# hbdat/cvpr22_cross_modal_pseudo_labeling

Measured on AMD Instinct MI355X. Metric: images/sec student-teacher train step (COCO 800x1333), higher is better.
Workload: dtype f32 (bf16x3 split MFMA, fp32 accum); 1 GPU; student_teacher_mask_rcnn_uncertainty.yaml R-50-C4, 2 img/GPU 3x800x1333, fwd+bwd+allreduce+SGD; global_batch=2, parallelism=dp1, losses_finite=True, pipelined=True

## Files before the change

### cvpr22_cross_modal_pseudo_labeling_amd/_C.py

```python
import contextlib
import functools
import ctypes
import threading

import torch

from . import _cpu, _lib

_L = _lib.load()


def _stream():
    return torch._C._cuda_getCurrentRawStream(torch.cuda.current_device())


class _Same:

    def __enter__(self):
        return None

    def __exit__(self, *exc):
        return False


# ... 737 lines not shown
        raise RuntimeError("im2col_nchw_pair: contiguous [N,C,H,W] float32 HIP tensor expected")
    n, c, h, w = x.shape
    ho, wo = (h + 2 * pad - kh) // stride + 1, (w + 2 * pad - kw) // stride + 1
    kp = -(-(kh * kw * c) // 32) * 32
    out = torch.empty((n * ho * wo, 2 * kp), dtype=torch.bfloat16, device=x.device)
    if out.numel():
        with _on(x.device):
            rc = _L.ovis_im2col_nchw_pair_f32(x.data_ptr(), out.data_ptr(), n, c, h, w, kh, kw, stride, pad, kp, _stream())
        _lib.check(rc, "im2col_nchw_pair")
    return out, (ho, wo)


_GEMM_TLS = threading.local()


@contextlib.contextmanager
def co_scheduled(on=True):
    prev = getattr(_GEMM_TLS, "co", False)
    _GEMM_TLS.co = bool(on)
    try:
        yield
    finally:
        _GEMM_TLS.co = prev


@functools.lru_cache(maxsize=None)
def _gemm_ws_bytes(m, n, ch, ch2, kh, kw, w, config):
    return int(_L.ovis_split_gemm_pair_workspace_bytes_ex(m, n, ch, ch2, kh, kw, w, config))


@functools.lru_cache(maxsize=None)
def _tn_slices(m, n, ch, taps):
    return int(_L.ovis_split_gemm_tn_slices(m, n, ch, taps))


@functools.lru_cache(maxsize=None)
def _gemm_f32_ws_bytes(m, n, k):
    return int(_L.ovis_gemm_f32_workspace_bytes(m, n, k))


@functools.lru_cache(maxsize=None)
def _nms_presorted_ws_bytes(n, k):
    return int(_L.ovis_nms_presorted_workspace_bytes(n, k))


@functools.lru_cache(maxsize=None)
def _topk_ws_bytes(n, a):
    return int(_L.ovis_topk_sorted_workspace_bytes(n, a))


def _gemm_cfg(config):
    return config | (0x10000 if getattr(_GEMM_TLS, "co", False) else 0)


def split_gemm_pair(a_pair, b_pair, bias=None, residual=None, relu=False, out_f32=True, out_pair=False, conv=None,
                    config=0, a2_pair=None, residual_pair=None):
    for t, name in ((a_pair, "a_pair"), (b_pair, "b_pair")) + (((a2_pair, "a2_pair"),) if a2_pair is not None else ()):
        if not (t.is_cuda and t.dtype == torch.bfloat16 and t.dim() == 2 and t.stride(1) == 1):
            raise RuntimeError(f"split_gemm_pair: {name} must be a 2-D bfloat16 HIP tensor in pair layout")
    m, ch = a_pair.shape[0], a_pair.shape[1] // 2
    n, k = b_pair.shape[0], b_pair.shape[1] // 2
    ch2 = 0
    if a2_pair is not None:
        if conv is not None or a2_pair.shape[0] != m:
            raise RuntimeError("split_gemm_pair: a2_pair needs a plain product and as many rows as a_pair")
        ch2 = a2_pair.shape[1] // 2
# ... 148 lines not shown
                                              0 if cp is None else cp.data_ptr(), 4 * n, residual_pair.data_ptr(),
                                              2 * residual_pair.stride(0), gate_pair.data_ptr(), 2 * gate_pair.stride(0), m, n,
                                              ch, config, _stream())
    _lib.check(rc, "split_gemm_pair_rp_gated")
    return c, cp


def split_gemm_pair_tn_supported(n, ch, conv=None):
    if n % 128 or ch % 128:
        return False
    if conv is not None:
        h, w, kh, kw = conv
        return kh % 2 == 1 and kw % 2 == 1
    return True


def split_gemm_pair_tn(g_pair, x_pair, conv=None, scale=None, weight_shape=None):
    for t, name in ((g_pair, "g_pair"), (x_pair, "x_pair")):
        if not (t.is_cuda and t.dtype == torch.bfloat16 and t.dim() == 2 and t.stride(1) == 1):
            raise RuntimeError(f"split_gemm_pair_tn: {name} must be a 2-D bfloat16 HIP tensor in pair layout")
    m, n, ch = g_pair.shape[0], g_pair.shape[1] // 2, x_pair.shape[1] // 2
    if x_pair.shape[0] != m:
        raise RuntimeError("split_gemm_pair_tn: row counts differ")
    h = w = 0
    kh = kw = 1
    if conv is not None:
        h, w, kh, kw = conv
        if m % (h * w):
            raise RuntimeError("split_gemm_pair_tn: rows must be a multiple of h*w")
    dev = g_pair.device
    if m == 0:
        z = torch.zeros((n, kh * kw * ch), dtype=torch.float32, device=dev)
        return z if weight_shape is None else z.new_zeros(weight_shape)
    slices = _tn_slices(m, n, ch, kh * kw)
    slabs = torch.empty((slices, n, kh * kw * ch), dtype=torch.float32, device=dev)
    with _on(dev):
        rc = _L.ovis_split_gemm_pair_tn(g_pair.data_ptr(), 2 * g_pair.stride(0), x_pair.data_ptr(), 2 * x_pair.stride(0),
                                        slabs.data_ptr(), slices, m, n, ch, kh, kw, h, w, _stream())
        _lib.check(rc, "split_gemm_pair_tn")
        if weight_shape is None:
            return slabs[0] if slices == 1 else slabs.sum(0)
        if tuple(weight_shape) != (n, ch, kh, kw):
            raise RuntimeError("split_gemm_pair_tn: weight_shape must be (N, ch, kh, kw)")
        dw = torch.empty(weight_shape, dtype=torch.float32, device=dev)
        if scale is not None:
            scale = _dev(scale.detach(), "scale")
        rc = _L.ovis_slab_reduce_f32(slabs.data_ptr(), 0 if scale is None else scale.data_ptr(), dw.data_ptr(), slices, n,
                                     ch, kh * kw, _stream())
    _lib.check(rc, "slab_reduce")
    return dw


def bias_act_(y, bias=None, residual=None, relu=True):
    if not (y.is_cuda and y.dtype == torch.float32 and y.dim() == 2 and y.is_contiguous()):
        raise RuntimeError("bias_act_: contiguous 2-D float32 HIP tensor expected")
    if residual is not None and not (residual.is_contiguous() and residual.shape == y.shape):
        raise RuntimeError("bias_act_: residual must be contiguous with y's shape")
    if y.numel() == 0:
        return y
    with _on(y.device):
        rc = _L.ovis_bias_act_f32(y.data_ptr(), 0 if bias is None else bias.data_ptr(),
                                  0 if residual is None else residual.data_ptr(), y.shape[0], y.shape[1],
                                  int(bool(relu)), _stream())
    _lib.check(rc, "bias_act")
    return y


# ... 552 lines not shown
```

### cvpr22_cross_modal_pseudo_labeling_amd/_lib.py

```python
import ctypes
import os

_HERE = os.path.dirname(os.path.abspath(__file__))
LIB_PATH = os.path.join(_HERE, "libovis_hip.so")

OVIS_OK = 0
_ERRORS = {-1: "OVIS_EINVAL (bad size or null pointer)",
           -2: "OVIS_ENOSPC (workspace too small)",
           -3: "OVIS_ERANGE (problem size not supported by the kernel)"}

_vp, _i, _f, _sz, _l = ctypes.c_void_p, ctypes.c_int, ctypes.c_float, ctypes.c_size_t, ctypes.c_long

SIGNATURES = {
    "ovis_version": (ctypes.c_char_p, []),
    "ovis_roi_align_forward_f32": (_i, [_vp, _vp, _vp, _i, _i, _i, _i, _i, _i, _i, _f, _i, _vp]),
    "ovis_roi_align_forward_workspace_bytes": (_sz, [_i, _i, _i]),
    "ovis_roi_align_forward_mfma_supported": (_i, [_i, _i, _i, _i]),
    "ovis_roi_align_forward_ws_f32": (_i, [_vp, _vp, _vp, _i, _i, _i, _i, _i, _i, _i, _f, _i, _vp, _sz, _vp]),
    "ovis_roi_align_forward_strided_from_nhwc_f32": (_i, [_vp, _vp, _vp, _i, _i, _i, _i, _i, _i, _i, _i, _f, _i, _i, _vp]),
    "ovis_roi_align_backward_f32": (_i, [_vp, _vp, _vp, _i, _i, _i, _i, _i, _i, _i, _f, _i, _vp]),
    "ovis_roi_align_backward_workspace_bytes": (_sz, [_i, _i, _i, _i]),
    "ovis_roi_align_backward_plane_supported": (_i, [_i, _i, _i, _i]),
    "ovis_roi_align_backward_ws_f32": (_i, [_vp, _vp, _vp, _i, _i, _i, _i, _i, _i, _i, _f, _i, _vp, _sz, _vp]),
    "ovis_roi_align_backward_strided_ws_f32": (_i, [_vp, _vp, _vp, _i, _i, _i, _i, _i, _i, _i, _i, _f, _i, _vp, _sz, _vp]),
# ... 3 lines not shown
    "ovis_roi_pool_backward_f32": (_i, [_vp, _vp, _vp, _vp, _i, _i, _i, _i, _i, _i, _i, _vp]),
    "ovis_deform_psroi_pool_forward_f32": (_i, [_vp] * 5 + [_i] * 7 + [_f] + [_i] * 5 + [_f, _vp]),
    "ovis_deform_psroi_pool_backward_f32": (_i, [_vp] * 7 + [_i] * 7 + [_f] + [_i] * 5 + [_f, _vp]),
    "ovis_nms_workspace_bytes": (_sz, [_i]),
    "ovis_nms_f32": (_i, [_vp, _vp, _i, _f, _i, _vp, _sz, _vp, _vp, _vp]),
    "ovis_nms_grouped_f32": (_i, [_vp, _vp, _vp, _i, _f, _i, _vp, _sz, _vp, _vp, _vp]),
    "ovis_sample_fg_bg": (_i, [_vp, _i, _i, _i, ctypes.c_uint64, _vp, _vp, _vp, _vp]),
    "ovis_project_pasted_masks_f32": (_i, [_vp, _vp, _vp, _vp, _i, _i, _i, _i, _i, _f, _vp, _vp]),
    "ovis_paste_masks_u8": (_i, [_vp, _vp, _i, _i, _i, _i, _f, _vp, _vp]),
    "ovis_render_instances_u8": (_i, [_vp, _i, _i, _vp, _vp, _i, _i, _vp, _vp, _vp, _f, _vp, _i, _vp, _vp]),
    "ovis_nms_presorted_workspace_bytes": (_sz, [_i, _i]),
    "ovis_nms_presorted_batched_f32": (_i, [_vp, _vp, _i, _i, _f, _i, _i, _vp, _sz, _vp, _vp, _vp]),
    "ovis_box_decode_f32": (_i, [_vp, _l, _vp, _l, _l, _i, _f, _f, _f, _f, _f, _i, _vp, _vp, _vp, _vp]),
    "ovis_smooth_l1_picked_fwd_bwd_f32": (_i, [_vp, _l, _i, _i, _vp, _l, _vp, _vp, _i, _i, _f, _f, _vp, _vp, _vp]),
    "ovis_gather_rows": (_i, [_vp, _i, _vp, _vp, _vp, _vp, _vp, _vp, _vp, _vp, _vp]),
    "ovis_rois_from_boxes_f32": (_i, [_vp, _vp, _vp, _i, _vp, _vp]),
    "ovis_deform_conv_implicit_f32": (_i, [_vp, _vp, _vp, _vp, _l, _vp, _vp, _l] + [_i] * 16 + [_vp]),
    "ovis_topk_sorted_workspace_bytes": (_sz, [_i, _i]),
    "ovis_topk_sorted_f32": (_i, [_vp, _l, _i, _i, _i, _vp, _vp, _vp, _sz, _vp]),
    "ovis_rpn_decode_f32": (_i, [_vp, _l, _l, _l, _vp, _vp, _vp, _i, _i, _i, _i, _f, _f, _f, _f, _f, _f, _f, _vp, _vp, _vp]),
    "ovis_sigmoid_focal_loss_forward_f32": (_i, [_vp, _vp, _vp, _i, _i, _f, _f, _vp]),
    "ovis_sigmoid_focal_loss_backward_f32": (_i, [_vp, _vp, _vp, _vp, _i, _i, _f, _f, _vp]),
    "ovis_split_bf16x3_f32": (_i, [_vp, _l, _vp, _l, _i, _i, _vp]),
    "ovis_im2col_split_bf16x3_f32": (_i, [_vp, _vp, _l, _i, _i, _i, _i, _i, _i, _vp]),
    "ovis_bias_act_f32": (_i, [_vp, _vp, _vp, _l, _i, _i, _vp]),
    "ovis_split_pair_f32": (_i, [_vp, _l, _vp, _l, _i, _vp]),
    "ovis_gate_split_pair_rows_f32": (_i, [_vp, _l, _vp, _i, _vp, _vp, _l, _i, _vp, _i, _vp, _vp, _vp]),
    "ovis_gate_split_pair_f32": (_i, [_vp, _l, _vp, _i, _vp, _vp, _l, _i, _vp, _i, _vp]),
    "ovis_im2col_nchw_pair_f32": (_i, [_vp, _vp] + [_i] * 9 + [_vp]),
    "ovis_weight_prep_pair_f32": (_i, [_vp, _vp, _vp, _vp, _i, _i, _i, _vp]),
    "ovis_slab_reduce_f32": (_i, [_vp, _vp, _vp, _i, _i, _i, _i, _vp]),
    "ovis_im2col_pair": (_i, [_vp, _vp, _l, _i, _i, _i, _i, _i, _vp]),
    "ovis_split_gemm_tn_slices": (_i, [_l, _i, _i, _i]),
    "ovis_split_gemm_pair_tn": (_i, [_vp, _l, _vp, _l, _vp, _i, _l, _i, _i, _i, _i, _i, _i, _vp]),
    "ovis_split_gemm_pair_gated": (_i, [_vp, _l, _vp, _l, _vp, _l, _vp, _l, _vp, _l, _l] + [_i] * 8 + [_vp]),
    "ovis_split_gemm_pair_gated_ws": (_i, [_vp, _l, _vp, _l, _vp, _l, _vp, _l, _vp, _l, _l] + [_i] * 7 + [_vp, _sz, _i, _vp]),
    "ovis_split_gemm_pair_workspace_bytes": (_sz, [_l, _i, _i, _i, _i, _i, _i]),
    "ovis_split_gemm_pair_workspace_bytes_ex": (_sz, [_l, _i, _i, _i, _i, _i, _i, _i]),
    "ovis_split_gemm_pair_rp_gated": (_i, [_vp, _l, _vp, _l, _vp, _l, _vp, _l, _vp, _l, _vp, _l, _l, _i, _i, _i, _vp]),
    "ovis_split_gemm_pair_pool_supported": (_i, [_l, _i, _i, _i]),
    "ovis_split_gemm_pair_rp_pool": (_i, [_vp, _l, _vp, _l, _vp, _l, _vp, _l, _vp, _vp, _l, _l, _i, _i, _i, _vp, _i, _f, _vp]),
    "ovis_split_gemm_pair_rp": (_i, [_vp, _l, _vp, _l, _vp, _l, _vp, _l, _vp, _vp, _l, _l, _i, _i, _i, _vp, _sz, _i, _vp]),
    "ovis_split_gemm_pair": (_i, [_vp, _l, _vp, _l, _vp, _l, _vp, _l, _vp, _l, _vp, _vp, _l, _l] + [_i] * 9
                             + [_vp, _sz, _i, _vp]),
    "ovis_match_encode_f32": (_i, [_vp, _vp, _vp, _i, _i, _f, _f, _i, _f, _f, _f, _f, _vp, _vp, _vp, _vp]),
    "ovis_rpn_match_encode_f32": (_i, [_vp, _vp, _vp, _i, _i, _f, _f, _i, _f, _f, _f, _f, _vp, _vp, _vp, _vp]),
    "ovis_project_masks_f32": (_i, [_vp, _vp, _vp, _i, _i, _i, _i, _i, _vp, _vp]),
    "ovis_gemm_f32": (_i, [_vp, _l, _l, _vp, _l, _l, _vp, _vp, _l, _i, _i, _i, _vp]),
    "ovis_gemm_ex_f32": (_i, [_vp, _l, _l, _vp, _l, _l, _vp, _i, _f, _i, _vp, _l, _i, _i, _i, _vp]),
    "ovis_gemm_f32_workspace_bytes": (_sz, [_i, _i, _i]),
    "ovis_gemm_ex_ws_f32": (_i, [_vp, _l, _l, _vp, _l, _l, _vp, _i, _f, _i, _vp, _l, _i, _i, _i, _vp, _sz, _vp]),
    "ovis_deform_im2col_f32": (_i, [_vp, _vp, _vp, _vp] + [_i] * 13 + [_vp]),
    "ovis_deform_col2im_f32": (_i, [_vp, _vp, _vp, _vp] + [_i] * 13 + [_vp]),
    "ovis_deform_col2im_coord_f32": (_i, [_vp, _vp, _vp, _vp, _vp, _vp] + [_i] * 13 + [_vp]),
    "ovis_deform_im2col_pair_rows_f32": (_i, [_vp, _vp, _vp, _vp, _l] + [_i] * 15 + [_vp]),
    "ovis_deform_col2im_rows_f32": (_i, [_vp, _l, _vp, _vp, _vp, _vp, _vp, _vp] + [_i] * 15 + [_vp]),
    "ovis_region_noun_align_f32": (_i, [_vp, _vp, _vp, _vp, _vp, _i, _i, _i, _vp]),
    "ovis_text_embed_f32": (_i, [_vp, _l, _i, _vp, _vp, _i, _i, _vp, _vp]),
    "ovis_project_polygon_masks_f32": (_i, [_vp, _vp, _vp, _vp, _vp, _i, _i, _i, _i, _vp, _vp]),
    "ovis_polygons_to_masks_workspace_bytes": (_sz, [_i, _i, _i]),
    "ovis_polygons_to_masks_u8": (_i, [_vp, _vp, _vp, _i, _i, _i, _i, _vp, _sz, _vp, _vp]),
    "ovis_transform_images_workspace_bytes": (_sz, [_i, _i, _i]),
    "ovis_transform_images_u8": (_i, [_vp, _l, _vp, _i, _i, _i, _vp, _vp, _i, _i, _i, _vp, _sz, _vp, _vp]),
    "ovis_sgd_momentum_multi_f32": (_i, [_vp, _vp, _i, _f, _f, _f, _i, _vp]),
    "ovis_bottleneck_identity_backward_workspace_bytes": (_sz, [_l, _i, _i, _i, _i, _i, _i]),
    "ovis_bottleneck_identity_backward": (_i, [_vp, _l] * 7 + [_vp] * 3 + [_l, _i, _i, _i, _i, _i, _i] + [_vp] * 7 + [_sz, _i, _vp, _vp]),
# ... 38 lines not shown
```

### cvpr22_cross_modal_pseudo_labeling_amd/csrc/bottleneck_backward.hip

```cpp
#include "ovis_common.h"

namespace {

inline size_t bb_align(size_t v) { return (v + 255) & ~(size_t)255; }

struct BbPlan {
  size_t chain_bytes;
  size_t slab_bytes;
  int s1, s2, s3;
};

BbPlan bb_plan(long m, int cin, int mid, int kh, int kw, int width, int config) {
  BbPlan p;
  const size_t a = ovis_split_gemm_pair_workspace_bytes_ex(m, mid, cin, 0, 1, 1, 0, config);
  const size_t b = ovis_split_gemm_pair_workspace_bytes_ex(m, mid, mid, 0, kh, kw, width, config);
  p.chain_bytes = bb_align(a > b ? a : b);
  p.s3 = ovis_split_gemm_tn_slices(m, cin, mid, 1);
  p.s2 = ovis_split_gemm_tn_slices(m, mid, mid, kh * kw);
  p.s1 = ovis_split_gemm_tn_slices(m, mid, cin, 1);
  const size_t w3 = (size_t)p.s3 * cin * mid * 4, w2 = (size_t)p.s2 * mid * mid * kh * kw * 4, w1 = (size_t)p.s1 * mid * cin * 4;
  size_t mx = w3 > w2 ? w3 : w2;
  if (w1 > mx) mx = w1;
  p.slab_bytes = bb_align(mx);
  return p;
}

hipEvent_t* bb_events() {
  static hipEvent_t ev[4];
  static bool made = false;
  if (!made) {
    for (int i = 0; i < 4; ++i)
      if (hipEventCreateWithFlags(&ev[i], hipEventDisableTiming) != hipSuccess) return nullptr;
    made = true;
  }
  return ev;
}

}

extern "C" size_t ovis_bottleneck_identity_backward_workspace_bytes(long m, int channels, int mid_channels, int taps_h,
                                                                    int taps_w, int width, int config) {
  if (m <= 0 || channels <= 0 || mid_channels <= 0 || taps_h <= 0 || taps_w <= 0) return 0;
  const BbPlan p = bb_plan(m, channels, mid_channels, taps_h, taps_w, width, config);
  return p.chain_bytes + p.slab_bytes;
}

extern "C" int ovis_bottleneck_identity_backward(
    const void* g3_pair, long g3_row_bytes, const void* x_pair, long x_row_bytes, const void* o1_pair, long o1_row_bytes,
    const void* o2_pair, long o2_row_bytes, const void* t1_pair, long t1_row_bytes, const void* t2_pair, long t2_row_bytes,
    const void* t3_pair, long t3_row_bytes, const float* scale1, const float* scale2, const float* scale3, long m, int channels,
    int mid_channels, int taps_h, int taps_w, int height, int width, void* g2_pair, void* g1_pair, void* gx_pair, float* dw1,
    float* dw2, float* dw3, void* workspace, size_t workspace_bytes, int config, void* stream, void* side_stream) {
  if (m <= 0 || channels <= 0 || mid_channels <= 0 || taps_h <= 0 || taps_w <= 0) return OVIS_EINVAL;
  if (!g3_pair || !x_pair || !o1_pair || !o2_pair || !t1_pair || !t2_pair || !t3_pair || !g2_pair || !g1_pair || !gx_pair ||
      !dw1 || !dw2 || !dw3 || !workspace)
    return OVIS_EINVAL;
  if (channels % 128 || mid_channels % 128 || !(taps_h & 1) || !(taps_w & 1)) return OVIS_ERANGE;
  const BbPlan p = bb_plan(m, channels, mid_channels, taps_h, taps_w, width, config);
  if (workspace_bytes < p.chain_bytes + p.slab_bytes) return OVIS_ENOSPC;
  hipStream_t s = (hipStream_t)stream;
  hipStream_t side = side_stream ? (hipStream_t)side_stream : s;
  const bool two = side != s;
  hipEvent_t* ev = two ? bb_events() : nullptr;
  if (two && !ev) return OVIS_EINVAL;
  char* chain_ws = (char*)workspace;
  float* slabs = (float*)((char*)workspace + p.chain_bytes);
  const int cin = channels, mid = mid_channels, taps = taps_h * taps_w;
  int rc;
#define BB_TRY(call)            \
  do {                          \
    rc = (call);                \
    if (rc != OVIS_OK) return rc; \
  } while (0)
#define BB_AFTER_MAIN(i)                                              \
  if (two) {                                                          \
    OVIS_HIP_TRY(hipEventRecord(ev[i], s));                           \
    OVIS_HIP_TRY(hipStreamWaitEvent(side, ev[i], 0));                 \
  }
  BB_AFTER_MAIN(0)
  BB_TRY(ovis_split_gemm_pair_tn(g3_pair, g3_row_bytes, o2_pair, o2_row_bytes, slabs, p.s3, m, cin, mid, 1, 1, 0, 0, side));
  BB_TRY(ovis_slab_reduce_f32(slabs, scale3, dw3, p.s3, cin, mid, 1, side));
  BB_TRY(ovis_split_gemm_pair_gated_ws(g3_pair, g3_row_bytes, t3_pair, t3_row_bytes, nullptr, mid, g2_pair, 4L * mid, o2_pair,
                                       o2_row_bytes, m, mid, cin, 1, 1, 0, 0, 0, chain_ws, p.chain_bytes, config, s));
  BB_AFTER_MAIN(1)
  BB_TRY(ovis_split_gemm_pair_tn(g2_pair, 4L * mid, o1_pair, o1_row_bytes, slabs, p.s2, m, mid, mid, taps_h, taps_w, height,
                                 width, side));
  BB_TRY(ovis_slab_reduce_f32(slabs, scale2, dw2, p.s2, mid, mid, taps, side));
  BB_TRY(ovis_split_gemm_pair_gated_ws(g2_pair, 4L * mid, t2_pair, t2_row_bytes, nullptr, mid, g1_pair, 4L * mid, o1_pair,
                                       o1_row_bytes, m, mid, mid, taps_h, taps_w, height, width, 1, chain_ws, p.chain_bytes,
                                       config, s));
  BB_AFTER_MAIN(2)
// ... 13 lines not shown
```

### cvpr22_cross_modal_pseudo_labeling_amd/csrc/split_gemm.hip

```cpp
#include <stdlib.h>

#include "ovis_common.h"
constexpr int kGroupWidth = 4;

namespace {
typedef short bf16x8 __attribute__((ext_vector_type(8)));
typedef float f32x4 __attribute__((ext_vector_type(4)));
typedef __bf16 b2 __attribute__((ext_vector_type(2)));
typedef float f2 __attribute__((ext_vector_type(2)));

__device__ char g_zero_line[128];

enum { PLAIN = 0, SHIFTED = 1, HALO = 2, DEFORM = 3 };
constexpr int kHalo = 8;

struct SplitGemmArgs {
  const char* A; long a_rs;
  const char* A2; long a2_rs;
  const char* B; long b_rs;
  float* C; long ldc;
  char* Cp; long cp_rs;
  const float* bias; const float* res; long ldr;
  const char* resp; long resp_rs;
  const char* gate; long gate_rs;
  float* pool; int pool_rows; float pool_scale;
  float* slab;
  long M; int N; int ch; int ch2; int T; int H; int W; int KH; int KW; int flip; int relu; int gw;
  int kslices; int steps_per_slice;
  const float* dimg; const float* doff; const float* dmask;
  int Ho; int Wo; int sh; int sw; int ph; int pw; int dlh; int dlw; int dg;
};

__device__ __forceinline__ void glds16(const char* gsrc, char* lds_wave_base) {
// ... 470 lines not shown
      if (er == 0 && col_ok && first < p.M && (sgm == 0 || (sgm == 1 ? pool_b1 : pool_b2) < 64)) {
        float* d = p.pool + (pool_map0 + sgm) * p.N + n;
#pragma unroll
        for (int e = 0; e < 4; ++e) atomicAdd(d + e, v[e] * p.pool_scale);
      }
    }
  }
}

__global__ __launch_bounds__(256) void split_gemm_finish_kernel(SplitGemmArgs p) {
  const int n4 = p.N >> 2;
  const long total = p.M * n4;
  const long slab = p.M * p.N;
  for (long i = (long)blockIdx.x * 256 + threadIdx.x; i < total; i += (long)gridDim.x * 256) {
    const long m = i / n4;
    const int n = (int)(i - m * n4) * 4;
    const float* s = p.slab + m * p.N + n;
    f32x4 v = *(const f32x4*)s;
    for (int k = 1; k < p.kslices; ++k) v += *(const f32x4*)(s + k * slab);
    epilogue_store4(p, m, n, v);
  }
}

typedef short bf16x4 __attribute__((ext_vector_type(4)));

struct SplitGemmTnArgs {
  const char* G; long g_rs;
  const char* X; long x_rs;
  float* C;
  long M; int N; int ch; int T; int H; int W; int KH; int KW; int slices; int steps_per_slice;
  int g_major;
};

#define OVIS_TR_READ(dst, addr, off) \
  asm volatile("ds_read_b64_tr_b16 %0, %1 offset:%2" : "=v"(dst) : "v"(addr), "n"(off) : "memory")
#define OVIS_LGKM_WAIT8(N, a, b, c, d, e, f, g, h)                                                                \
  asm volatile("s_waitcnt lgkmcnt(%8)"                                                                             \
               : "+v"(a), "+v"(b), "+v"(c), "+v"(d), "+v"(e), "+v"(f), "+v"(g), "+v"(h)                            \
               : "n"(N)                                                                                            \
               : "memory")

template <bool CONV, bool SMALL = false>
__global__ __launch_bounds__(256, 2) void split_gemm_tn_kernel(SplitGemmTnArgs p, int tiles_i, int tiles_j,
                                                              int nblocks) {
  constexpr int TILE_BYTES = 32 * 512, STAGE = 2 * TILE_BYTES;
  extern __shared__ __attribute__((aligned(16))) char smem[];
  const int lane = threadIdx.x & 63, wave = threadIdx.x >> 6;
  int id;
  {
    constexpr int kChunk = 2 * OVIS_NUM_CU;
    const int b = blockIdx.x, base = b / kChunk * kChunk;
    const int nb = min(nblocks - base, kChunk), bl = b - base;
    const int q = nb >> 3, r = nb & 7, xcd = bl & 7, loc = bl >> 3;
    id = base + (xcd < r ? xcd * (q + 1) : r * (q + 1) + (xcd - r) * q) + loc;
  }
  const int per_slice = tiles_i * tiles_j;
  const int slice = id / per_slice;
  const int rem = id - slice * per_slice;
  const int tile_j = p.g_major ? rem % tiles_j : rem / tiles_i;
  const int tile_i = p.g_major ? rem / tiles_j : rem - tile_j * tiles_i;
  const int i0 = tile_i * 128, j0 = tile_j * 128;
  const int tap = CONV ? j0 / p.ch : 0, c0 = CONV ? j0 - tap * p.ch : j0;
  int off_rows = 0, tdy = 0, tdx = 0;
  if (CONV) {
    tdy = tap / p.KW - p.KH / 2;
    tdx = tap % p.KW - p.KW / 2;
    off_rows = tdy * p.W + tdx;
  }
  const long step0 = (long)slice * p.steps_per_slice;
  const long steps_total = (p.M + 31) >> 5;
  long step1 = step0 + p.steps_per_slice;
  if (step1 > steps_total) step1 = steps_total;
  const int nk = step1 > step0 ? (int)(step1 - step0) : 0;

  const int prow = lane >> 5, pseg = (lane & 31) >> 1, phalf = lane & 1;
  int rows[4];
  long g_off[4], x_off[4];
  int x_y[4], x_x[4];
  int m_row[4];
  const int HW = CONV ? p.H * p.W : 1;
  unsigned long long tap_mask = 0;
  if (CONV && SMALL) {
    const int qy = lane / p.W, qx = lane - qy * p.W;
    tap_mask = __ballot(lane < HW && (unsigned)(qy + tdy) < (unsigned)p.H && (unsigned)(qx + tdx) < (unsigned)p.W);
  }
#pragma unroll
  for (int i = 0; i < 4; ++i) {
    const int piece = wave * 4 + i;
    const int row = piece * 2 + prow;
    rows[i] = row;
    const int fr = (((row >> 3) & 1) << 2) | (row & 3);
    const int seg = pseg ^ fr;
    const int m = (int)(step0 << 5) + row;
    m_row[i] = m;
    g_off[i] = (long)m * p.g_rs + (long)i0 * 4 + seg * 32 + phalf * 16;
    x_off[i] = ((long)m + off_rows) * p.x_rs + (long)c0 * 4 + seg * 32 + phalf * 16;
    x_x[i] = CONV ? (SMALL ? m % HW : m % p.W) : 0;
    x_y[i] = (CONV && !SMALL) ? (m / p.W) % p.H : 0;
  }
  const int step_q = (CONV && SMALL) ? 32 % HW : 0;
  const int step_dx = CONV ? 32 % p.W : 0, step_dy = CONV ? 32 / p.W : 0;
  const bool y_single = step_dy + 1 <= p.H;
  const char* zero_src = g_zero_line + (lane & 7) * 16;
  const int Mi = (int)p.M;

  auto issue = [&](int stage) {
    char* base = smem + stage * STAGE;
    bool x_ok[4];
#pragma unroll
    for (int i = 0; i < 4; ++i) {
      x_ok[i] = m_row[i] < Mi;
      if (CONV && SMALL) {
        x_ok[i] = x_ok[i] && ((tap_mask >> x_x[i]) & 1ull) != 0ull;
        int q = x_x[i] + step_q;
        if (q >= HW) q -= HW;
        x_x[i] = q;
      } else if (CONV) {
        x_ok[i] = x_ok[i] && (unsigned)(x_y[i] + tdy) < (unsigned)p.H && (unsigned)(x_x[i] + tdx) < (unsigned)p.W;
        int x = x_x[i] + step_dx, y = x_y[i] + step_dy;
        if (x >= p.W) { x -= p.W; ++y; }
        if (y_single) { if (y >= p.H) y -= p.H; } else { y %= p.H; }
        x_x[i] = x;
        x_y[i] = y;
      }
    }
#pragma unroll
    for (int i = 0; i < 4; ++i) {
      const char* src = p.G + g_off[i];
      if (m_row[i] >= Mi) src = zero_src;
      glds16(src, base + (wave * 4 + i) * 1024);
      g_off[i] += 32 * p.g_rs;
    }
#pragma unroll
    for (int i = 0; i < 4; ++i) {
      const char* src = p.X + x_off[i];
      if (!x_ok[i]) src = zero_src;
      glds16(src, base + TILE_BYTES + (wave * 4 + i) * 1024);
      x_off[i] += 32 * p.x_rs;
      m_row[i] += 32;
    }
  };

  const int wi = wave >> 1, wj = wave & 1;
  const int gq = lane >> 4, pp = lane & 15;
  const int rrow = 8 * gq + (pp >> 2);
  const int rfr = ((gq & 1) << 2) | (pp >> 2);
  int g_rd[4], x_rd[4];
#pragma unroll
  for (int f = 0; f < 4; ++f) {
    const int seg_g = (2 * wi + (f >> 1)) * 4 + (f & 1);
    g_rd[f] = rrow * 512 + ((seg_g ^ rfr) << 5) + (pp & 3) * 8;
    const int seg_x = (2 * wj + (f >> 1)) * 4 + (f & 1);
    x_rd[f] = TILE_BYTES + rrow * 512 + ((seg_x ^ rfr) << 5) + (pp & 3) * 8;
  }

  f32x4 acc[4][4];
#pragma unroll
  for (int f = 0; f < 4; ++f)
#pragma unroll
    for (int g = 0; g < 4; ++g) acc[f][g] = f32x4{0.f, 0.f, 0.f, 0.f};

  if (nk > 0) issue(0);
  for (int kb = 0; kb < nk; ++kb) {
    __syncthreads();
    if (kb + 1 < nk) issue((kb + 1) & 1);
    const int so = (kb & 1) * STAGE;
    bf16x4 xa[4][2], xb[4][2], ga[4][2], gb[4][2];
#pragma unroll
    for (int f = 0; f < 4; ++f) {
      const int ax = so + x_rd[f], ag = so + g_rd[f];
      OVIS_TR_READ(xa[f][0], ax, 0);
      OVIS_TR_READ(xb[f][0], ax, 2048);
      OVIS_TR_READ(ga[f][0], ag, 0);
// ... 391 lines not shown
                     (char*)dst_pair, num * height * width, height, width, channels, kh, kw);
  OVIS_LAUNCH_CHECK();
  return OVIS_OK;
}

extern "C" int ovis_split_gemm_tn_slices(long m, int n, int channels, int taps) {
  if (m <= 0 || n <= 0 || channels <= 0 || taps <= 0) return 1;
  const long tiles = (long)(n / 128) * ((long)taps * channels / 128);
  const long steps = (m + 31) / 32;
  if (tiles <= 0) return 1;
  const long slots = 2L * OVIS_NUM_CU;
  if (steps >= 128 && steps <= 1100 && tiles <= 64) {
    long s = slots / tiles;
    if (s > steps / 16) s = steps / 16;
    if (s > 256) s = 256;
    return (int)(s < 1 ? 1 : s);
  }
  long s_max = (4 * slots + tiles - 1) / tiles;
  if (s_max > steps / 8) s_max = steps / 8;
  if (s_max > 256) s_max = 256;
  if (s_max < 1) s_max = 1;
  long best = 1;
  double best_score = -1.0;
  for (long s = 1; s <= s_max; ++s) {
    const long blocks = s * tiles, rounds = (blocks + slots - 1) / slots;
    double score = (double)blocks / (double)(rounds * slots);
    if (rounds == 1) score *= 0.97 * (double)blocks / (double)slots;
    if (rounds > 2) score -= 0.01 * (double)(rounds - 2);
    if (score > best_score + 1e-9) { best_score = score; best = s; }
  }
  return (int)best;
}

extern "C" int ovis_split_gemm_pair_tn(const void* g_pair, long g_row_bytes, const void* x_pair, long x_row_bytes,
                                       float* c_slabs, int slices, long m, int n, int channels, int taps_h,
                                       int taps_w, int height, int width, void* stream) {
  if (m < 0 || n <= 0 || channels <= 0 || taps_h <= 0 || taps_w <= 0 || !(taps_h & 1) || !(taps_w & 1) || slices <= 0)
    return OVIS_EINVAL;
  if (!g_pair || !x_pair || !c_slabs || m > 0x7fffff00L) return OVIS_EINVAL;
  const int T = taps_h * taps_w;
  if (T > 1 && (height <= 0 || width <= 0)) return OVIS_EINVAL;
  if (n % 128 != 0 || channels % 128 != 0 ||
      g_row_bytes % 16 != 0 || x_row_bytes % 16 != 0 || ((uintptr_t)g_pair & 15) || ((uintptr_t)x_pair & 15) ||
      ((uintptr_t)c_slabs & 15))
    return OVIS_ERANGE;
  SplitGemmTnArgs p;
  p.G = (const char*)g_pair; p.g_rs = g_row_bytes; p.X = (const char*)x_pair; p.x_rs = x_row_bytes;
  p.C = c_slabs; p.M = m; p.N = n; p.ch = channels; p.T = T; p.H = height; p.W = width; p.KH = taps_h; p.KW = taps_w;
  p.slices = slices;
  const long steps = (m + 31) / 32;
  p.steps_per_slice = (int)((steps + slices - 1) / slices);
  const int tiles_i = n / 128, tiles_j = (int)((long)T * channels / 128);
  p.g_major = tiles_i >= channels / 128 ? 1 : 0;
  const long nblocks = (long)tiles_i * tiles_j * slices;
  if (nblocks > 0x7fffffffL) return OVIS_ERANGE;
  hipStream_t s = (hipStream_t)stream;
  const int lds = 2 * 2 * 32 * 512;
  if (T > 1 && (long)height * width <= 64) {
    static bool attr_set_s = false;
    if (!attr_set_s) {
      OVIS_HIP_TRY(hipFuncSetAttribute((const void*)split_gemm_tn_kernel<true, true>, hipFuncAttributeMaxDynamicSharedMemorySize, lds));
      attr_set_s = true;
    }
    hipLaunchKernelGGL((split_gemm_tn_kernel<true, true>), dim3((unsigned)nblocks), dim3(256), lds, s, p, tiles_i, tiles_j, (int)nblocks);
  } else if (T > 1) {
    static bool attr_set_c = false;
    if (!attr_set_c) {
      OVIS_HIP_TRY(hipFuncSetAttribute((const void*)split_gemm_tn_kernel<true>, hipFuncAttributeMaxDynamicSharedMemorySize, lds));
      attr_set_c = true;
    }
    hipLaunchKernelGGL(split_gemm_tn_kernel<true>, dim3((unsigned)nblocks), dim3(256), lds, s, p, tiles_i, tiles_j, (int)nblocks);
  } else {
    static bool attr_set = false;
    if (!attr_set) {
      OVIS_HIP_TRY(hipFuncSetAttribute((const void*)split_gemm_tn_kernel<false>, hipFuncAttributeMaxDynamicSharedMemorySize, lds));
      attr_set = true;
    }
    hipLaunchKernelGGL(split_gemm_tn_kernel<false>, dim3((unsigned)nblocks), dim3(256), lds, s, p, tiles_i, tiles_j, (int)nblocks);
  }
  OVIS_LAUNCH_CHECK();
  return OVIS_OK;
}

namespace {
struct SplitGemmPlan {
  int mode, narrow, stages, kslices, steps_per_slice, tiles_m, tiles_n;
};

SplitGemmPlan split_gemm_plan(long m, int n, int channels, int channels2, int taps_h, int taps_w, int width, int config) {
  SplitGemmPlan q;
  const int T = taps_h * taps_w;
  q.narrow = n <= 64;
  const int bn = q.narrow ? 64 : 128;
  q.tiles_m = (int)((m + 127) / 128);
  q.tiles_n = (n + bn - 1) / bn;
  const long nb = (long)q.tiles_m * q.tiles_n;
  q.mode = PLAIN;
  if (T > 1) q.mode = (!q.narrow && !(config & 4) && (taps_h / 2) * width + taps_w / 2 <= kHalo && T <= 16) ? HALO : SHIFTED;
  const int cpb = channels / 32;
  const int units = q.mode == HALO ? cpb : T * cpb + channels2 / 32;
  q.kslices = 1;
  q.steps_per_slice = units;
  bool sliced_two_stage = false;
  if (!(config & 8) && !q.narrow && nb <= OVIS_NUM_CU / 2) {
    const int min_units = q.mode == HALO ? 1 : 8;
    long s = units / min_units;
    const long want = (2L * OVIS_NUM_CU + nb - 1) / nb;
    if (s > want) s = want;
    if (s > 64) s = 64;
    if (s >= 2) {
      q.steps_per_slice = (int)((units + s - 1) / s);
// ... 275 lines not shown
```

### include/ovis_hip.h

```cpp
#ifndef OVIS_HIP_H_
#define OVIS_HIP_H_

#include <stddef.h>
#include <stdint.h>

#ifdef __cplusplus
extern "C" {
#endif

#define OVIS_OK 0
#define OVIS_EINVAL (-1)
#define OVIS_ENOSPC (-2)
#define OVIS_ERANGE (-3)

const char* ovis_version(void);

int ovis_roi_align_forward_f32(const float* input, const float* rois, float* output,
                               int num_rois, int batch, int channels, int height,
                               int width, int pooled_h, int pooled_w,
                               float spatial_scale, int sampling_ratio, void* stream);

size_t ovis_roi_align_forward_workspace_bytes(int num_rois, int height, int width);
int ovis_roi_align_forward_mfma_supported(int height, int width, int pooled_h, int pooled_w);
int ovis_roi_align_forward_ws_f32(const float* input, const float* rois, float* output,
// ... 128 lines not shown
                               float* c, long ldc, void* c_pair, long c_pair_row_bytes, const void* gate_pair,
                               long gate_row_bytes, long m, int n, int channels, int taps_h, int taps_w,
                               int height, int width, int flip, int config, void* stream);

int ovis_split_gemm_pair_gated_ws(const void* a_pair, long a_row_bytes, const void* b_pair, long b_row_bytes,
                                  float* c, long ldc, void* c_pair, long c_pair_row_bytes, const void* gate_pair,
                                  long gate_row_bytes, long m, int n, int channels, int taps_h, int taps_w,
                                  int height, int width, int flip, void* workspace, size_t workspace_bytes,
                                  int config, void* stream);

int ovis_split_gemm_pair_rp_gated(const void* a_pair, long a_row_bytes, const void* b_pair, long b_row_bytes, float* c,
                                  long ldc, void* c_pair, long c_pair_row_bytes, const void* residual_pair,
                                  long residual_pair_row_bytes, const void* gate_pair, long gate_row_bytes, long m, int n,
                                  int channels, int config, void* stream);

int ovis_im2col_nchw_pair_f32(const float* src, void* dst_pair, int num, int channels, int height, int width,
                              int kh, int kw, int stride, int pad, int k_padded, void* stream);

size_t ovis_split_gemm_pair_workspace_bytes(long m, int n, int channels, int channels2, int taps_h, int taps_w,
                                            int width);
size_t ovis_split_gemm_pair_workspace_bytes_ex(long m, int n, int channels, int channels2, int taps_h, int taps_w,
                                               int width, int config);
int ovis_split_gemm_pair(const void* a_pair, long a_row_bytes, const void* a2_pair, long a2_row_bytes,
                         const void* b_pair, long b_row_bytes, float* c, long ldc, void* c_pair,
                         long c_pair_row_bytes, const float* bias, const float* residual, long ldr, long m,
                         int n, int channels, int channels2, int taps_h, int taps_w, int height, int width,
                         int flip, int relu, void* workspace, size_t workspace_bytes, int config, void* stream);
int ovis_split_gemm_pair_rp(const void* a_pair, long a_row_bytes, const void* b_pair, long b_row_bytes, float* c, long ldc,
                            void* c_pair, long c_pair_row_bytes, const float* bias, const void* residual_pair,
                            long residual_pair_row_bytes, long m, int n, int channels, int relu, void* workspace,
                            size_t workspace_bytes, int config, void* stream);

int ovis_split_gemm_tn_slices(long m, int n, int channels, int taps);
int ovis_split_gemm_pair_tn(const void* g_pair, long g_row_bytes, const void* x_pair, long x_row_bytes,
                            float* c_slabs, int slices, long m, int n, int channels, int taps_h,
                            int taps_w, int height, int width, void* stream);

int ovis_match_encode_f32(const float* gt_boxes, const int64_t* gt_labels, const float* proposals, int num_gt,
                          int num_proposals, float high_threshold, float low_threshold, int between_keeps_label,
                          float wx, float wy, float ww, float wh, int64_t* matched_idx, int64_t* labels,
                          float* regression_targets, void* stream);
int ovis_rpn_match_encode_f32(const float* gt_boxes, const float* anchors, const uint8_t* visibility, int num_gt,
                              int num_anchors, float high_threshold, float low_threshold, int allow_low_quality_matches,
                              float wx, float wy, float ww, float wh, uint32_t* best_per_gt_scratch, int64_t* labels,
                              float* regression_targets, void* stream);
int ovis_project_masks_f32(const uint8_t* masks, const int64_t* gt_index, const float* boxes, int num, int height,
                           int width, int resolution, int masks_are_bool, float* out, void* stream);
int ovis_sample_fg_bg(const int64_t* labels, int num, int batch_size, int max_positives, uint64_t seed,
                      int64_t* selected, int64_t* positive_slots, int32_t* counts, void* stream);
int ovis_project_pasted_masks_f32(const float* mask_probs, const float* gt_boxes, const int64_t* gt_index,
                                  const float* boxes, int num, int image_height, int image_width, int prob_resolution,
                                  int resolution, float threshold, float* out, void* stream);
int ovis_paste_masks_u8(const float* mask_probs, const float* boxes, int num, int prob_resolution, int image_height,
                        int image_width, float threshold, uint8_t* out, void* stream);
int ovis_render_instances_u8(const uint8_t* image, int height, int width, const float* maps, const float* boxes,
                             int num_layers, int map_resolution, const int32_t* kinds, const float* params,
                             const float* colors, float alpha, const uint8_t* outline_colors, int outline_thickness,
                             uint8_t* out, void* stream);
int ovis_gather_rows(const int64_t* index, int num, const float* boxes_a, float* boxes_a_out, const float* boxes_b,
                     float* boxes_b_out, const int64_t* ints_a, int64_t* ints_a_out, const int64_t* ints_b,
                     int64_t* ints_b_out, void* stream);

int ovis_gemm_f32(const float* A, long a_row_stride, long a_k_stride, const float* B,
                  long b_row_stride, long b_k_stride, const float* bias, float* C,
                  long c_row_stride, int M, int N, int K, void* stream);

// ... 115 lines not shown
```

Baseline: 60.34 images/sec.

## Skip out-of-bounds rows per tap in small-map conv weight-gradient GEMM

For conv weight gradients on small feature maps (at most 64 pixels, e.g. ROI-head 7x7/14x14), the TN GEMM now iterates only over each tap's valid pixel window instead of all rows with masked zero loads. Taps are grouped into classes by valid-pixel count, blocks are laid out per class, and the slice count comes from a makespan simulation that balances per-class work against slab-reduce cost. This removes loads and MFMA steps spent on padded positions, at the cost of extra index arithmetic (magic division) and more complex block-to-tile mapping.

```diff
diff --git a/cvpr22_cross_modal_pseudo_labeling_amd/_C.py b/cvpr22_cross_modal_pseudo_labeling_amd/_C.py
--- a/cvpr22_cross_modal_pseudo_labeling_amd/_C.py
+++ b/cvpr22_cross_modal_pseudo_labeling_amd/_C.py
@@ -793,6 +793,11 @@
 @functools.lru_cache(maxsize=None)
 def _tn_slices(m, n, ch, taps):
     return int(_L.ovis_split_gemm_tn_slices(m, n, ch, taps))
+
+
+@functools.lru_cache(maxsize=None)
+def _tn_map_slices(m, n, ch, kh, kw, h, w):
+    return int(_L.ovis_split_gemm_tn_map_slices(m, n, ch, kh, kw, h, w))
 
 
 @functools.lru_cache(maxsize=None)
@@ -1007,7 +1012,7 @@
     if m == 0:
         z = torch.zeros((n, kh * kw * ch), dtype=torch.float32, device=dev)
         return z if weight_shape is None else z.new_zeros(weight_shape)
-    slices = _tn_slices(m, n, ch, kh * kw)
+    slices = _tn_slices(m, n, ch, 1) if conv is None else _tn_map_slices(m, n, ch, kh, kw, h, w)
     slabs = torch.empty((slices, n, kh * kw * ch), dtype=torch.float32, device=dev)
     with _on(dev):
         rc = _L.ovis_split_gemm_pair_tn(g_pair.data_ptr(), 2 * g_pair.stride(0), x_pair.data_ptr(), 2 * x_pair.stride(0),
diff --git a/cvpr22_cross_modal_pseudo_labeling_amd/_lib.py b/cvpr22_cross_modal_pseudo_labeling_amd/_lib.py
--- a/cvpr22_cross_modal_pseudo_labeling_amd/_lib.py
+++ b/cvpr22_cross_modal_pseudo_labeling_amd/_lib.py
@@ -59,6 +59,7 @@
     "ovis_slab_reduce_f32": (_i, [_vp, _vp, _vp, _i, _i, _i, _i, _vp]),
     "ovis_im2col_pair": (_i, [_vp, _vp, _l, _i, _i, _i, _i, _i, _vp]),
     "ovis_split_gemm_tn_slices": (_i, [_l, _i, _i, _i]),
+    "ovis_split_gemm_tn_map_slices": (_i, [_l, _i, _i, _i, _i, _i, _i]),
     "ovis_split_gemm_pair_tn": (_i, [_vp, _l, _vp, _l, _vp, _i, _l, _i, _i, _i, _i, _i, _i, _vp]),
     "ovis_split_gemm_pair_gated": (_i, [_vp, _l, _vp, _l, _vp, _l, _vp, _l, _vp, _l, _l] + [_i] * 8 + [_vp]),
     "ovis_split_gemm_pair_gated_ws": (_i, [_vp, _l, _vp, _l, _vp, _l, _vp, _l, _vp, _l, _l] + [_i] * 7 + [_vp, _sz, _i, _vp]),
diff --git a/cvpr22_cross_modal_pseudo_labeling_amd/csrc/bottleneck_backward.hip b/cvpr22_cross_modal_pseudo_labeling_amd/csrc/bottleneck_backward.hip
--- a/cvpr22_cross_modal_pseudo_labeling_amd/csrc/bottleneck_backward.hip
+++ b/cvpr22_cross_modal_pseudo_labeling_amd/csrc/bottleneck_backward.hip
@@ -10,13 +10,21 @@
   int s1, s2, s3;
 };
 
-BbPlan bb_plan(long m, int cin, int mid, int kh, int kw, int width, int config) {
+BbPlan bb_plan(long m, int cin, int mid, int kh, int kw, int height, int width, int config) {
   BbPlan p;
   const size_t a = ovis_split_gemm_pair_workspace_bytes_ex(m, mid, cin, 0, 1, 1, 0, config);
   const size_t b = ovis_split_gemm_pair_workspace_bytes_ex(m, mid, mid, 0, kh, kw, width, config);
   p.chain_bytes = bb_align(a > b ? a : b);
   p.s3 = ovis_split_gemm_tn_slices(m, cin, mid, 1);
-  p.s2 = ovis_split_gemm_tn_slices(m, mid, mid, kh * kw);
+  if (height > 0) {
+    p.s2 = ovis_split_gemm_tn_map_slices(m, mid, mid, kh, kw, height, width);
+  } else {
+    p.s2 = ovis_split_gemm_tn_slices(m, mid, mid, kh * kw);
+    for (int h = 1; width > 0 && (long)h * width <= 64; ++h) {
+      const int s = ovis_split_gemm_tn_map_slices(m, mid, mid, kh, kw, h, width);
+      if (s > p.s2) p.s2 = s;
+    }
+  }
   p.s1 = ovis_split_gemm_tn_slices(m, mid, cin, 1);
   const size_t w3 = (size_t)p.s3 * cin * mid * 4, w2 = (size_t)p.s2 * mid * mid * kh * kw * 4, w1 = (size_t)p.s1 * mid * cin * 4;
   size_t mx = w3 > w2 ? w3 : w2;
@@ -41,7 +49,7 @@
 extern "C" size_t ovis_bottleneck_identity_backward_workspace_bytes(long m, int channels, int mid_channels, int taps_h,
                                                                     int taps_w, int width, int config) {
   if (m <= 0 || channels <= 0 || mid_channels <= 0 || taps_h <= 0 || taps_w <= 0) return 0;
-  const BbPlan p = bb_plan(m, channels, mid_channels, taps_h, taps_w, width, config);
+  const BbPlan p = bb_plan(m, channels, mid_channels, taps_h, taps_w, 0, width, config);
   return p.chain_bytes + p.slab_bytes;
 }
 
@@ -56,7 +64,7 @@
       !dw1 || !dw2 || !dw3 || !workspace)
     return OVIS_EINVAL;
   if (channels % 128 || mid_channels % 128 || !(taps_h & 1) || !(taps_w & 1)) return OVIS_ERANGE;
-  const BbPlan p = bb_plan(m, channels, mid_channels, taps_h, taps_w, width, config);
+  const BbPlan p = bb_plan(m, channels, mid_channels, taps_h, taps_w, height, width, config);
   if (workspace_bytes < p.chain_bytes + p.slab_bytes) return OVIS_ENOSPC;
   hipStream_t s = (hipStream_t)stream;
   hipStream_t side = side_stream ? (hipStream_t)side_stream : s;
diff --git a/cvpr22_cross_modal_pseudo_labeling_amd/csrc/split_gemm.hip b/cvpr22_cross_modal_pseudo_labeling_amd/csrc/split_gemm.hip
--- a/cvpr22_cross_modal_pseudo_labeling_amd/csrc/split_gemm.hip
+++ b/cvpr22_cross_modal_pseudo_labeling_amd/csrc/split_gemm.hip
@@ -1,4 +1,9 @@
 #include <stdlib.h>
+
+#include <functional>
+#include <mutex>
+#include <queue>
+#include <vector>
 
 #include "ovis_common.h"
 constexpr int kGroupWidth = 4;
@@ -535,6 +540,15 @@
   int g_major;
 };
 
+constexpr int kTnMaxTaps = 25, kTnMaxClasses = 9;
+struct TnMapPlan {
+  int R;
+  int ncls;
+  int cls_end[kTnMaxClasses];
+  int cls_tap0[kTnMaxClasses + 1];
+  unsigned char tap_of[kTnMaxTaps + 7];
+};
+
 #define OVIS_TR_READ(dst, addr, off) \
   asm volatile("ds_read_b64_tr_b16 %0, %1 offset:%2" : "=v"(dst) : "v"(addr), "n"(off) : "memory")
 #define OVIS_LGKM_WAIT8(N, a, b, c, d, e, f, g, h)                                                                \
@@ -544,24 +558,43 @@
                : "memory")
 
 template <bool CONV, bool SMALL = false>
-__global__ __launch_bounds__(256, 2) void split_gemm_tn_kernel(SplitGemmTnArgs p, int tiles_i, int tiles_j,
-                                                              int nblocks) {
+__global__ __launch_bounds__(256, 2) void split_gemm_tn_kernel(SplitGemmTnArgs p, TnMapPlan plan, int tiles_i,
+                                                              int tiles_j, int nblocks) {
   constexpr int TILE_BYTES = 32 * 512, STAGE = 2 * TILE_BYTES;
   extern __shared__ __attribute__((aligned(16))) char smem[];
   const int lane = threadIdx.x & 63, wave = threadIdx.x >> 6;
-  int id;
-  {
+  int id, slice, tile_i, tile_j;
+  if (CONV && SMALL) {
+    constexpr int kChunk = 2 * OVIS_NUM_CU;
+    const int b = blockIdx.x;
+    int k = 0;
+    while (k + 1 < plan.ncls && b >= plan.cls_end[k]) ++k;
+    const int cs = k ? plan.cls_end[k - 1] : 0, ce = plan.cls_end[k];
+    const int lo = cs + (b - cs) / kChunk * kChunk, hi = min(ce, lo + kChunk), xcd = b & 7;
+    int run = 0;
+    for (int x = 0; x < xcd; ++x) run += ((hi - x + 7) >> 3) - ((lo - x + 7) >> 3);
+    id = lo - cs + run + ((b - lo - ((xcd - lo) & 7)) >> 3);
+    const int ct = p.ch >> 7;
+    const int tiles_jc = (plan.cls_tap0[k + 1] - plan.cls_tap0[k]) * ct;
+    const int per_slice = tiles_i * tiles_jc;
+    slice = id / per_slice;
+    const int rem = id - slice * per_slice;
+    const int tjc = p.g_major ? rem % tiles_jc : rem / tiles_i;
+    tile_i = p.g_major ? rem / tiles_jc : rem - tjc * tiles_i;
+    const int ti = tjc / ct;
+    tile_j = plan.tap_of[plan.cls_tap0[k] + ti] * ct + (tjc - ti * ct);
+  } else {
     constexpr int kChunk = 2 * OVIS_NUM_CU;
     const int b = blockIdx.x, base = b / kChunk * kChunk;
     const int nb = min(nblocks - base, kChunk), bl = b - base;
     const int q = nb >> 3, r = nb & 7, xcd = bl & 7, loc = bl >> 3;
     id = base + (xcd < r ? xcd * (q + 1) : r * (q + 1) + (xcd - r) * q) + loc;
-  }
-  const int per_slice = tiles_i * tiles_j;
-  const int slice = id / per_slice;
-  const int rem = id - slice * per_slice;
-  const int tile_j = p.g_major ? rem % tiles_j : rem / tiles_i;
-  const int tile_i = p.g_major ? rem / tiles_j : rem - tile_j * tiles_i;
+    const int per_slice = tiles_i * tiles_j;
+    slice = id / per_slice;
+    const int rem = id - slice * per_slice;
+    tile_j = p.g_major ? rem % tiles_j : rem / tiles_i;
+    tile_i = p.g_major ? rem / tiles_j : rem - tile_j * tiles_i;
+  }
   const int i0 = tile_i * 128, j0 = tile_j * 128;
   const int tap = CONV ? j0 / p.ch : 0, c0 = CONV ? j0 - tap * p.ch : j0;
   int off_rows = 0, tdy = 0, tdx = 0;
@@ -570,55 +603,91 @@
     tdx = tap % p.KW - p.KW / 2;
     off_rows = tdy * p.W + tdx;
   }
-  const long step0 = (long)slice * p.steps_per_slice;
-  const long steps_total = (p.M + 31) >> 5;
-  long step1 = step0 + p.steps_per_slice;
+  const int HW = CONV ? p.H * p.W : 1;
+  int cnt = 0, wv = 1, pix0 = 0;
+  if (CONV && SMALL) {
+    const int hv = max(p.H - abs(tdy), 0);
+    wv = max(p.W - abs(tdx), 0);
+    cnt = hv * wv;
+    pix0 = max(-tdy, 0) * p.W + max(-tdx, 0);
+  }
+  const long steps_total = (CONV && SMALL) ? ((long)plan.R * cnt + 31) >> 5 : (p.M + 31) >> 5;
+  const int steps_per_slice = (CONV && SMALL) ? (int)((steps_total + p.slices - 1) / p.slices) : p.steps_per_slice;
+  const long step0 = (long)slice * steps_per_slice;
+  long step1 = step0 + steps_per_slice;
   if (step1 > steps_total) step1 = steps_total;
   const int nk = step1 > step0 ? (int)(step1 - step0) : 0;
 
   const int prow = lane >> 5, pseg = (lane & 31) >> 1, phalf = lane & 1;
-  int rows[4];
   long g_off[4], x_off[4];
   int x_y[4], x_x[4];
   int m_row[4];
-  const int HW = CONV ? p.H * p.W : 1;
-  unsigned long long tap_mask = 0;
-  if (CONV && SMALL) {
-    const int qy = lane / p.W, qx = lane - qy * p.W;
-    tap_mask = __ballot(lane < HW && (unsigned)(qy + tdy) < (unsigned)p.H && (unsigned)(qx + tdx) < (unsigned)p.W);
-  }
+  int col_off[4];
+  int pix[4], map0[4];
+  const int cntd = cnt > 0 ? cnt : 1;
 #pragma unroll
   for (int i = 0; i < 4; ++i) {
     const int piece = wave * 4 + i;
     const int row = piece * 2 + prow;
-    rows[i] = row;
     const int fr = (((row >> 3) & 1) << 2) | (row & 3);
     const int seg = pseg ^ fr;
     const int m = (int)(step0 << 5) + row;
-    m_row[i] = m;
-    g_off[i] = (long)m * p.g_rs + (long)i0 * 4 + seg * 32 + phalf * 16;
-    x_off[i] = ((long)m + off_rows) * p.x_rs + (long)c0 * 4 + seg * 32 + phalf * 16;
-    x_x[i] = CONV ? (SMALL ? m % HW : m % p.W) : 0;
-    x_y[i] = (CONV && !SMALL) ? (m / p.W) % p.H : 0;
-  }
-  const int step_q = (CONV && SMALL) ? 32 % HW : 0;
+    col_off[i] = seg * 32 + phalf * 16;
+    if (CONV && SMALL) {
+      const int r = m / cntd;
+      pix[i] = m - r * cntd;
+      map0[i] = r * HW;
+    } else {
+      m_row[i] = m;
+      g_off[i] = (long)m * p.g_rs + (long)i0 * 4 + col_off[i];
+      x_off[i] = ((long)m + off_rows) * p.x_rs + (long)c0 * 4 + col_off[i];
+      x_x[i] = CONV ? m % p.W : 0;
+      x_y[i] = CONV ? (m / p.W) % p.H : 0;
+    }
+  }
+  const int step_pix = 32 % cntd, step_map = 32 / cntd * HW;
+  const int wv_magic = (65536 + wv - 1) / max(wv, 1);
+  const int wgap = p.W - wv;
   const int step_dx = CONV ? 32 % p.W : 0, step_dy = CONV ? 32 / p.W : 0;
   const bool y_single = step_dy + 1 <= p.H;
   const char* zero_src = g_zero_line + (lane & 7) * 16;
   const int Mi = (int)p.M;
-
-  auto issue = [&](int stage) {
+  const unsigned g_rs32 = (unsigned)p.g_rs, x_rs32 = (unsigned)p.x_rs;
+  const char *g_col[4], *x_col[4];
+#pragma unroll
+  for (int i = 0; i < 4; ++i) {
+    g_col[i] = p.G + (long)i0 * 4 + col_off[i];
+    x_col[i] = p.X + (long)off_rows * p.x_rs + (long)c0 * 4 + col_off[i];
+  }
+
+  auto issue_small = [&](int stage) {
+    char* base = smem + stage * STAGE;
+    const char *gs[4], *xs[4];
+#pragma unroll
+    for (int i = 0; i < 4; ++i) {
+      const int y = (pix[i] * wv_magic) >> 16;
+      const int m = map0[i] + pix0 + pix[i] + y * wgap;
+      const bool ok = map0[i] < Mi;
+      gs[i] = ok ? g_col[i] + (unsigned long)(unsigned)m * g_rs32 : zero_src;
+      xs[i] = ok ? x_col[i] + (unsigned long)(unsigned)m * x_rs32 : zero_src;
+      int q = pix[i] + step_pix, r0 = map0[i] + step_map;
+      if (q >= cnt) { q -= cnt; r0 += HW; }
+      pix[i] = q;
+      map0[i] = r0;
+    }
+#pragma unroll
+    for (int i = 0; i < 4; ++i) glds16(gs[i], base + (wave * 4 + i) * 1024);
+#pragma unroll
+    for (int i = 0; i < 4; ++i) glds16(xs[i], base + TILE_BYTES + (wave * 4 + i) * 1024);
+  };
+
+  auto issue_rows = [&](int stage) {
     char* base = smem + stage * STAGE;
     bool x_ok[4];
 #pragma unroll
     for (int i = 0; i < 4; ++i) {
       x_ok[i] = m_row[i] < Mi;
-      if (CONV && SMALL) {
-        x_ok[i] = x_ok[i] && ((tap_mask >> x_x[i]) & 1ull) != 0ull;
-        int q = x_x[i] + step_q;
-        if (q >= HW) q -= HW;
-        x_x[i] = q;
-      } else if (CONV) {
+      if (CONV) {
         x_ok[i] = x_ok[i] && (unsigned)(x_y[i] + tdy) < (unsigned)p.H && (unsigned)(x_x[i] + tdx) < (unsigned)p.W;
         int x = x_x[i] + step_dx, y = x_y[i] + step_dy;
         if (x >= p.W) { x -= p.W; ++y; }
@@ -642,6 +711,9 @@
       x_off[i] += 32 * p.x_rs;
       m_row[i] += 32;
     }
+  };
+  auto issue = [&](int stage) {
+    if (CONV && SMALL) issue_small(stage); else issue_rows(stage);
   };
 
   const int wi = wave >> 1, wj = wave & 1;
@@ -1099,6 +1171,94 @@
   return (int)best;
 }
 
+namespace {
+struct TnTapClasses {
+  int ncls;
+  int ntaps[kTnMaxClasses];
+  int cnt[kTnMaxClasses];
+  unsigned char tap_of[kTnMaxTaps + 7];
+};
+
+bool tn_map_form(long m, long g_row_bytes, long x_row_bytes, int taps_h, int taps_w, int height, int width) {
+  const int T = taps_h * taps_w;
+  return T > 1 && taps_h <= 5 && taps_w <= 5 && height > 0 && width > 0 && (long)height * width <= 64 &&
+         m % ((long)height * width) == 0 && m <= 0x7fff0000L && g_row_bytes >= 0 && g_row_bytes <= 0x7fffffffL &&
+         x_row_bytes >= 0 && x_row_bytes <= 0x7fffffffL;
+}
+
+void tn_tap_classes(int taps_h, int taps_w, int height, int width, TnTapClasses* c) {
+  const int T = taps_h * taps_w;
+  int cnt[kTnMaxTaps];
+  for (int t = 0; t < T; ++t) {
+    const int dy = t / taps_w - taps_h / 2, dx = t % taps_w - taps_w / 2;
+    const int hv = height - (dy < 0 ? -dy : dy), wv = width - (dx < 0 ? -dx : dx);
+    cnt[t] = hv > 0 && wv > 0 ? hv * wv : 0;
+    int k = t;
+    for (; k > 0 && cnt[c->tap_of[k - 1]] < cnt[t]; --k) c->tap_of[k] = c->tap_of[k - 1];
+    c->tap_of[k] = (unsigned char)t;
+  }
+  c->ncls = 0;
+  for (int k = 0; k < T; ++k) {
+    const int v = cnt[c->tap_of[k]];
+    if (c->ncls > 0 && c->cnt[c->ncls - 1] == v) { ++c->ntaps[c->ncls - 1]; continue; }
+    c->cnt[c->ncls] = v;
+    c->ntaps[c->ncls++] = 1;
+  }
+}
+
+long tn_map_makespan(const TnTapClasses& c, long maps, long tiles_per_tap, int slices, long slots) {
+  std::priority_queue<long, std::vector<long>, std::greater<long>> free_at;
+  long end = 0;
+  for (int k = 0; k < c.ncls; ++k) {
+    const long steps = (maps * c.cnt[k] + 31) / 32, len = (steps + slices - 1) / slices + 8;
+    for (long b = tiles_per_tap * c.ntaps[k] * slices; b > 0; --b) {
+      long t = len;
+      if ((long)free_at.size() >= slots) { t += free_at.top(); free_at.pop(); }
+      free_at.push(t);
+      if (t > end) end = t;
+    }
+  }
+  return end;
+}
+}
+
+extern "C" int ovis_split_gemm_tn_map_slices(long m, int n, int channels, int taps_h, int taps_w, int height, int width) {
+  if (m <= 0 || n <= 0 || channels <= 0 || taps_h <= 0 || taps_w <= 0) return 1;
+  if (!tn_map_form(m, 0, 0, taps_h, taps_w, height, width)) return ovis_split_gemm_tn_slices(m, n, channels, taps_h * taps_w);
+  struct Key { long m; int n, ch, kh, kw, h, w, slices; };
+  static std::mutex memo_mutex;
+  static std::vector<Key> memo;
+  {
+    std::lock_guard<std::mutex> lock(memo_mutex);
+    for (const Key& k : memo)
+      if (k.m == m && k.n == n && k.ch == channels && k.kh == taps_h && k.kw == taps_w && k.h == height && k.w == width)
+        return k.slices;
+  }
+  const long tiles_per_tap = (long)(n / 128) * (channels / 128), tiles = tiles_per_tap * taps_h * taps_w;
+  if (tiles <= 0) return 1;
+  TnTapClasses c;
+  tn_tap_classes(taps_h, taps_w, height, width, &c);
+  const long maps = m / ((long)height * width), slots = 2L * OVIS_NUM_CU;
+  const long steps = (maps * c.cnt[0] + 31) / 32;
+  long s_max = (4 * slots + tiles - 1) / tiles;
+  if (s_max > steps / 8) s_max = steps / 8;
+  if (s_max > 256) s_max = 256;
+  if (s_max < 1) s_max = 1;
+  const double slab_steps = (double)n * taps_h * taps_w * channels / 524288.0;
+  long best = 1;
+  double best_cost = -1.0;
+  for (long s = 1; s <= s_max; ++s) {
+    const double cost = (double)tn_map_makespan(c, maps, tiles_per_tap, (int)s, slots) + slab_steps * (double)s;
+    if (best_cost < 0.0 || cost < best_cost - 1e-9) { best_cost = cost; best = s; }
+  }
+  {
+    std::lock_guard<std::mutex> lock(memo_mutex);
+    if (memo.size() >= 256) memo.clear();
+    memo.push_back(Key{m, n, channels, taps_h, taps_w, height, width, (int)best});
+  }
+  return (int)best;
+}
+
 extern "C" int ovis_split_gemm_pair_tn(const void* g_pair, long g_row_bytes, const void* x_pair, long x_row_bytes,
                                        float* c_slabs, int slices, long m, int n, int channels, int taps_h,
                                        int taps_w, int height, int width, void* stream) {
@@ -1123,27 +1283,39 @@
   if (nblocks > 0x7fffffffL) return OVIS_ERANGE;
   hipStream_t s = (hipStream_t)stream;
   const int lds = 2 * 2 * 32 * 512;
-  if (T > 1 && (long)height * width <= 64) {
+  TnMapPlan plan = {};
+  if (tn_map_form(m, g_row_bytes, x_row_bytes, taps_h, taps_w, height, width)) {
+    TnTapClasses c;
+    tn_tap_classes(taps_h, taps_w, height, width, &c);
+    plan.R = (int)(m / ((long)height * width));
+    plan.ncls = c.ncls;
+    long end = 0;
+    for (int k = 0; k < c.ncls; ++k) {
+      plan.cls_tap0[k + 1] = plan.cls_tap0[k] + c.ntaps[k];
+      end += (long)tiles_i * (channels / 128) * c.ntaps[k] * slices;
+      plan.cls_end[k] = (int)end;
+    }
+    for (int t = 0; t < T; ++t) plan.tap_of[t] = c.tap_of[t];
     static bool attr_set_s = false;
     if (!attr_set_s) {
       OVIS_HIP_TRY(hipFuncSetAttribute((const void*)split_gemm_tn_kernel<true, true>, hipFuncAttributeMaxDynamicSharedMemorySize, lds));
       attr_set_s = true;
     }
-    hipLaunchKernelGGL((split_gemm_tn_kernel<true, true>), dim3((unsigned)nblocks), dim3(256), lds, s, p, tiles_i, tiles_j, (int)nblocks);
+    hipLaunchKernelGGL((split_gemm_tn_kernel<true, true>), dim3((unsigned)nblocks), dim3(256), lds, s, p, plan, tiles_i, tiles_j, (int)nblocks);
   } else if (T > 1) {
     static bool attr_set_c = false;
     if (!attr_set_c) {
       OVIS_HIP_TRY(hipFuncSetAttribute((const void*)split_gemm_tn_kernel<true>, hipFuncAttributeMaxDynamicSharedMemorySize, lds));
       attr_set_c = true;
     }
-    hipLaunchKernelGGL(split_gemm_tn_kernel<true>, dim3((unsigned)nblocks), dim3(256), lds, s, p, tiles_i, tiles_j, (int)nblocks);
+    hipLaunchKernelGGL(split_gemm_tn_kernel<true>, dim3((unsigned)nblocks), dim3(256), lds, s, p, plan, tiles_i, tiles_j, (int)nblocks);
   } else {
     static bool attr_set = false;
     if (!attr_set) {
       OVIS_HIP_TRY(hipFuncSetAttribute((const void*)split_gemm_tn_kernel<false>, hipFuncAttributeMaxDynamicSharedMemorySize, lds));
       attr_set = true;
     }
-    hipLaunchKernelGGL(split_gemm_tn_kernel<false>, dim3((unsigned)nblocks), dim3(256), lds, s, p, tiles_i, tiles_j, (int)nblocks);
+    hipLaunchKernelGGL(split_gemm_tn_kernel<false>, dim3((unsigned)nblocks), dim3(256), lds, s, p, plan, tiles_i, tiles_j, (int)nblocks);
   }
   OVIS_LAUNCH_CHECK();
   return OVIS_OK;
diff --git a/include/ovis_hip.h b/include/ovis_hip.h
--- a/include/ovis_hip.h
+++ b/include/ovis_hip.h
@@ -184,6 +184,7 @@
                             size_t workspace_bytes, int config, void* stream);
 
 int ovis_split_gemm_tn_slices(long m, int n, int channels, int taps);
+int ovis_split_gemm_tn_map_slices(long m, int n, int channels, int taps_h, int taps_w, int height, int width);
 int ovis_split_gemm_pair_tn(const void* g_pair, long g_row_bytes, const void* x_pair, long x_row_bytes,
                             float* c_slabs, int slices, long m, int n, int channels, int taps_h,
                             int taps_w, int height, int width, void* stream);
```

Measured after the change: 60.96 images/sec, median of 6. 1.01x the previous value.
